# HyTruongSon/GraphFlow

Hardware: AMD Instinct MI355X
Metric: CCN-2D (SMP_omega) molecules/sec fwd+bwd (higher is better)
Workload: dtype f32 (level block products: 2xf16-split operands, 22-bit, fp32 accumulate); 1 GPU; cfg3: SMP_omega 3 levels, C=64, F=5, D=5, cap=29, batch=1024 synthetic QM9-size molecules/GPU, device-resident, fused levels; parallelism=single GPU

## Files before the change

graphflow_amd/csrc/smp_level_c64_split.hip:

```cpp
#include <cstdlib>
#include <type_traits>

#include "gemm_lds.h"
#include "gf_internal.h"
#include "smp_internal.h"

namespace gf {
namespace {

using lds_image::f16v;
using lds_image::f4v;
typedef _Float16 h8 __attribute__((ext_vector_type(8)));
typedef _Float16 h2 __attribute__((ext_vector_type(2)));
typedef float f2v __attribute__((ext_vector_type(2)));

constexpr int kSpThreads = 512;

template <unsigned EMIN = 14u>
__device__ __forceinline__ void pow2_scale(unsigned maxbits, float *s, float *inv) {
    unsigned e = maxbits >> 23;
    e = e < EMIN ? EMIN : e;
    *s = __uint_as_float((267u - e) << 23);
    *inv = __uint_as_float((e - 13u) << 23);
}
// ... 458 lines not shown
    float *facs = winv + 16;
    const int tid = threadIdx.x, lane = tid & 63, li = lane & 31, lh = lane >> 5, wave = tid >> 6;
    for (int t = tid; t < NPOS * E; t += kSmThreads) {
        const int g = (pos0 + t / E) * 512 + t % E;
        imgH[t] = wimg[g];
        imgL[t] = wimg[kSpAll + g];
    }
    if (tid < NPOS) winv[tid] = reinterpret_cast<const float *>(wimg + 2 * kSpAll)[pos0 + tid];
    __syncthreads();
    float *myfac = facs + wave * 32;
    struct Raw {
        f4v a[VPL / 4];
    };
    struct Spl {
        uint4 h[NC], l[NC];
    };
    auto split_blk = [&](const Raw &R, Spl &S, float &inv) {
        unsigned m = 0u;
#pragma unroll
        for (int q = 0; q < VPL / 4; ++q)
#pragma unroll
            for (int j = 0; j < 4; ++j) {
                const unsigned b = __float_as_uint(R.a[q][j]) & 0x7fffffffu;
                m = b > m ? b : m;
            }
        const unsigned mo = (unsigned)__shfl_xor((int)m, 32);
        m = mo > m ? mo : m;
        float sc;
        pow2_scale(m, &sc, &inv);
#pragma unroll
        for (int c = 0; c < NC; ++c) {
            unsigned hw[4], lw[4];
#pragma unroll
            for (int j = 0; j < 4; ++j) {
                h2 h, l;
                const f4v v = R.a[2 * c + (j >> 1)];
                split_pair(v[2 * (j & 1)], v[2 * (j & 1) + 1], sc, &h, &l);
                hw[j] = __builtin_bit_cast(unsigned, h);
                lw[j] = __builtin_bit_cast(unsigned, l);
            }
            S.h[c] = make_uint4(hw[0], hw[1], hw[2], hw[3]);
            S.l[c] = make_uint4(lw[0], lw[1], lw[2], lw[3]);
        }
    };
    auto prod = [&](const Spl &S, float rowfac, int wpos, f16v &acc0, f16v &acc1) {
        __builtin_amdgcn_wave_barrier();
        myfac[li] = rowfac * winv[wpos];
        __builtin_amdgcn_wave_barrier();
        const uint4 *bh = imgH + (size_t)wpos * E + lane, *bl = imgL + (size_t)wpos * E + lane;
#pragma unroll
        for (int nh = 0; nh < NH; ++nh) {
            f16v t;
#pragma unroll
            for (int r = 0; r < 16; ++r) t[r] = 0.f;
#pragma unroll
            for (int c = 0; c < NC; ++c) {
                const h8 bhc = __builtin_bit_cast(h8, bh[(NC * nh + c) * 64]), blc = __builtin_bit_cast(h8, bl[(NC * nh + c) * 64]);
                const h8 ah = __builtin_bit_cast(h8, S.h[c]), al = __builtin_bit_cast(h8, S.l[c]);
                t = __builtin_amdgcn_mfma_f32_32x32x16_f16(al, bhc, t, 0, 0, 0);
                t = __builtin_amdgcn_mfma_f32_32x32x16_f16(ah, blc, t, 0, 0, 0);
            }
#pragma unroll
            for (int r = 0; r < 16; ++r) t[r] *= kLowUnscale;
#pragma unroll
            for (int c = 0; c < NC; ++c) {
                const h8 bhc = __builtin_bit_cast(h8, bh[(NC * nh + c) * 64]);
                const h8 ah = __builtin_bit_cast(h8, S.h[c]);
                t = __builtin_amdgcn_mfma_f32_32x32x16_f16(ah, bhc, t, 0, 0, 0);
            }
            f16v &acc = nh ? acc1 : acc0;
#pragma unroll
            for (int g = 0; g < 4; ++g) {
                const f4v fac = *reinterpret_cast<const f4v *>(myfac + 8 * g + 4 * lh);
#pragma unroll
                for (int j = 0; j < 4; ++j) acc[4 * g + j] += t[4 * g + j] * fac[j];
            }
        }
        __builtin_amdgcn_wave_barrier();
    };
    const int npanels = (rows + 31) / 32;
    for (int p = wg * (kSmThreads / 64) + wave; p < npanels; p += nwg * (kSmThreads / 64)) {
        const int r0 = p * 32;
        const int row = r0 + li < rows ? r0 + li : rows - 1;
        Raw R[NIN];
#pragma unroll
        for (int k = 0; k < NIN; ++k) {
            const float *src = In + (size_t)row * LDA + k * CB + VPL * lh;
#pragma unroll
            for (int q = 0; q < VPL / 4; ++q) R[k].a[q] = *reinterpret_cast<const f4v *>(src + 4 * q);
        }
        (void)NIN;
        auto store_out = [&](int o, const f16v &acc0, const f16v &acc1) {
            float *out = Out + (size_t)(r0 + 4 * lh) * LDOUT + o * CB + li;
#pragma unroll
            for (int r = 0; r < 16; ++r) {
                const int rr = (r & 3) + 8 * (r >> 2);
                if (r0 + 4 * lh + rr < rows && li < CB) {
                    out[(size_t)rr * LDOUT] = acc0[r];
                    if constexpr (NH == 2) out[(size_t)rr * LDOUT + 32] = acc1[r];
                }
            }
        };
        f16v acc0, acc1;
        Spl X;
        float iX;
        if constexpr (PROG == 0) {
#pragma unroll
            for (int r = 0; r < 16; ++r) acc0[r] = acc1[r] = 0.f;
#pragma unroll
            for (int k = 0; k < NPOS; ++k) {
                split_blk(R[k], X, iX);
                prod(X, iX, k, acc0, acc1);
            }
            store_out(0, acc0, acc1);
        } else if constexpr (PROG == 1) {
            split_blk(R[0], X, iX);
#pragma unroll
            for (int k = 0; k < NPOS; ++k) {
#pragma unroll
                for (int r = 0; r < 16; ++r) acc0[r] = acc1[r] = 0.f;
                prod(X, iX, k, acc0, acc1);
                store_out(k, acc0, acc1);
            }
        } else {
#pragma unroll
            for (int k = 0; k < NPOS; ++k) {
                split_blk(R[k], X, iX);
#pragma unroll
                for (int r = 0; r < 16; ++r) acc0[r] = acc1[r] = 0.f;
                prod(X, iX, k, acc0, acc1);
                store_out(k, acc0, acc1);
            }
        }
    }
}

template <int CB>
__global__ __launch_bounds__(kSmThreads, 2) void smp_small_split(SmallJobs jobs, const uint4 *__restrict__ wimg) {
    int j = 0;
    if (jobs.n > 1 && (int)blockIdx.x >= jobs.wg0[1]) j = 1;
    if (jobs.n > 2 && (int)blockIdx.x >= jobs.wg0[2]) j = 2;
    const int wg = (int)blockIdx.x - jobs.wg0[j];
    switch (jobs.prog[j]) {
        case 0: small_split_body<0, CB>(jobs.In[j], jobs.Out[j], jobs.rows[j], wimg, jobs.pos0[j], wg, jobs.nwg[j]); break;
        case 1: small_split_body<1, CB>(jobs.In[j], jobs.Out[j], jobs.rows[j], wimg, jobs.pos0[j], wg, jobs.nwg[j]); break;
        default: small_split_body<2, CB>(jobs.In[j], jobs.Out[j], jobs.rows[j], wimg, jobs.pos0[j], wg, jobs.nwg[j]); break;
    }
}

constexpr int kWsThreads = 512, kWsSlice = 16, kWsRowWords = 12;
constexpr int kWsACols = 256, kWsBCols = 320;
constexpr int kWsStageWords = 2 * (kWsACols + kWsBCols) * kWsRowWords;
constexpr size_t kWsLds = 2 * (size_t)kWsStageWords * 4 + 2 * (kWsACols + kWsBCols) * sizeof(float);
__constant__ int c_ws_ablk[8] = {0, 1, 0, 2, 3, 0, 1, 0};
__constant__ int c_ws_bblk[8] = {1, 1, 2, 0, 0, 3, 3, 4};

__global__ __launch_bounds__(kWsThreads, 1) void smp_wgrad_split(const float *__restrict__ T, const float *__restrict__ dO,
                                                                  const float *__restrict__ rs, int rows, int kchunk,
                                                                  float *__restrict__ part, const int *__restrict__ trow,
                                                                  const unsigned *__restrict__ cmax,
                                                                  const unsigned *__restrict__ chan,
                                                                  float smax, float max_tot, float max_tr,
                                                                  const unsigned *__restrict__ row_max,
                                                                  int packed) {
    extern __shared__ __attribute__((aligned(16))) unsigned ws_smem[];
    const int tid = threadIdx.x, lane = tid & 63, li = lane & 31, lg = lane >> 5;
    const int wave = __builtin_amdgcn_readfirstlane(tid >> 6);
    const int kend = rows;
    auto K = [&](int n) { return (long long)(blockIdx.x + (long long)n * gridDim.x) * kWsSlice; };

    float *sScale = reinterpret_cast<float *>(ws_smem + 2 * kWsStageWords), *sInv = sScale + kWsACols + kWsBCols;
    if (cmax) {
        for (int c = tid; c < kWsACols + kWsBCols; c += kWsThreads) pow2_scale_col(cmax[c], &sScale[c], &sInv[c]);
    } else {
        if (row_max) {
            max_tot = __uint_as_float(row_max[0]);
            max_tr = __uint_as_float(row_max[1]);
        }
        for (int c = tid; c < kWsACols + kWsBCols; c += kWsThreads) {
            const bool isa = c < kWsACols;
            const int blk = (isa ? c : c - kWsACols) >> 6, ch = c & 63;
            const float m = __uint_as_float(chan[(isa ? 0 : 64) + ch]);
            const float fa = blk < 2 ? smax : max_tot;
            const float fb = blk == 0 ? 1.f : blk == 2 ? max_tr : max_tot;
            pow2_scale_col(__float_as_uint(m * (isa ? fa : fb)), &sScale[c], &sInv[c]);
        }
    }
    __syncthreads();

    const int q_lo = lane & 7, pair = lane >> 3;
    struct Task {
        f4v v0, v1;
    };
    constexpr int NB = 2;
    struct Set {
        Task ta, tb[NB];
        float f0[NB], f1[NB];
    };
    const bool has_b1 = wave < 2;
    const int zbit = ((wave >> 1) & 1) == 0 ? 31 : 29;
    const int a_quad = 8 * wave + q_lo;
    auto b_blk = [&](int e) { return (wave + 8 * e) >> 1; };
    auto b_quad = [&](int e) { return 8 * ((wave + 8 * e) & 1) + q_lo; };
    const int rot = (q_lo >> 1) & 3;
    f4v a_scale, b_scale[NB];
#pragma unroll
    for (int i = 0; i < 4; ++i) {
        a_scale[i] = sScale[4 * a_quad + ((i + rot) & 3)];
#pragma unroll
        for (int e = 0; e < NB; ++e) {
            const int blk = b_blk(e) < 5 ? b_blk(e) : 0;
            b_scale[e][i] = sScale[kWsACols + 64 * blk + 4 * b_quad(e) + ((i + rot) & 3)];
        }
    }
    int ia0 = 0, ia1 = 0, ib0 = 0, ib1 = 0;
    auto fetch_trow = [&](int m, int &t0, int &t1) {
        const long long k = K(m) + 2 * pair, last = kend - 1;
        t0 = trow[k < last ? k : last];
        t1 = trow[k + 1 < last ? k + 1 : last];
    };
    auto load_slice = [&](Set &S, int m) {
        const int g0 = packed ? (ia0 & 0x1fffffff) : ia0, g1 = packed ? (ia1 & 0x1fffffff) : ia1;
        const bool z0 = packed && !((ia0 >> zbit) & 1), z1 = packed && !((ia1 >> zbit) & 1);
        const bool zg0 = packed && ia0 >= 0, zg1 = packed && ia1 >= 0;
        ia0 = ib0, ia1 = ib1;
        fetch_trow(m + 2, ib0, ib1);
        const long long last = kend - 1, kk = K(m) + 2 * pair;
        const int c0 = (int)(kk < last ? kk : last), c1 = (int)(kk + 1 < last ? kk + 1 : last);
        const float *t0 = T + (size_t)c0 * 256 + 4 * a_quad, *t1 = T + (size_t)c1 * 256 + 4 * a_quad;
        S.ta.v0 = gf_ld_s<4>(reinterpret_cast<const f4v *>(z0 ? sp_zero_page + 4 * q_lo : t0));
        S.ta.v1 = gf_ld_s<4>(reinterpret_cast<const f4v *>(z1 ? sp_zero_page + 4 * q_lo : t1));
#pragma unroll
        for (int e = 0; e < NB; ++e) {
            const int blk = b_blk(e);
            S.f0[e] = rs[(size_t)c0 * 2 + (blk == 2)];
            S.f1[e] = rs[(size_t)c1 * 2 + (blk == 2)];
            const bool gathered = blk == 4;
            const float *src = blk < 5 ? dO + (blk >= 3 ? 64 : 0) + 4 * b_quad(e) : T + 4 * a_quad;
            const int ld = blk < 5 ? 128 : 256;
            const float *s0 = src + (size_t)(gathered ? g0 : c0) * ld, *s1 = src + (size_t)(gathered ? g1 : c1) * ld;
            S.tb[e].v0 = gf_ld_s<256>(reinterpret_cast<const f4v *>((gathered && zg0) ? sp_zero_page + 4 * q_lo : s0));
            S.tb[e].v1 = gf_ld_s<256>(reinterpret_cast<const f4v *>((gathered && zg1) ? sp_zero_page + 4 * q_lo : s1));
        }
    };
    auto rotate = [&](f4v v) {
        if (rot & 1) v = f4v{v[1], v[2], v[3], v[0]};
        if (rot & 2) v = f4v{v[2], v[3], v[0], v[1]};
        return v;
    };
    auto store_task = [&](const f4v &v0, const f4v &v1, unsigned *H, unsigned *L, int col0, const f4v &sc, float f0, float f1) {
        const f4v r0 = rotate(v0), r1 = rotate(v1);
#pragma unroll
        for (int i = 0; i < 4; ++i) {
            h2 h, l;
            split_plain2(r0[i], r1[i], sc[i] * f0, sc[i] * f1, &h, &l);
            const int w = (col0 + ((i + rot) & 3)) * kWsRowWords + pair;
            H[w] = __builtin_bit_cast(unsigned, h);
            L[w] = __builtin_bit_cast(unsigned, l);
        }
    };
    auto store_slice = [&](const Set &S, long long k0, unsigned *stage) {
        unsigned *Ah = stage, *Al = Ah + kWsACols * kWsRowWords, *Bh = Al + kWsACols * kWsRowWords, *Bl = Bh + kWsBCols * kWsRowWords;
        const long long k = k0 + 2 * pair;
        const float ok0 = k < kend ? 1.f : 0.f, ok1 = k + 1 < kend ? 1.f : 0.f;
        store_task(S.ta.v0, S.ta.v1, Ah, Al, 4 * a_quad, a_scale, ok0, ok1);
#pragma unroll
        for (int e = 0; e < NB; ++e) {
            if (e == 1 && !has_b1) break;
            const int blk = b_blk(e);
            const bool scaled = blk == 1 || blk == 2;
            const float m0 = scaled ? S.f0[e] : 1.f, m1 = scaled ? S.f1[e] : 1.f;
            store_task(S.tb[e].v0, S.tb[e].v1, Bh, Bl, 64 * blk + 4 * b_quad(e), b_scale[e], ok0 * m0, ok1 * m1);
        }
    };

    f16v acc[2][2];
#pragma unroll
    for (int r = 0; r < 16; ++r) acc[0][0][r] = acc[0][1][r] = acc[1][0][r] = acc[1][1][r] = 0.f;
    const int ablk = c_ws_ablk[wave], bblk = c_ws_bblk[wave];
    auto products = [&](const unsigned *stage) {
        const unsigned *Ah = stage, *Al = Ah + kWsACols * kWsRowWords, *Bh = Al + kWsACols * kWsRowWords, *Bl = Bh + kWsBCols * kWsRowWords;
        const int ao = (ablk * 64 + li) * kWsRowWords + 4 * lg, bo = (bblk * 64 + li) * kWsRowWords + 4 * lg;
        h8 ah[2], al[2], bh[2], bl[2];
#pragma unroll
        for (int t = 0; t < 2; ++t) {
            ah[t] = __builtin_bit_cast(h8, *reinterpret_cast<const uint4 *>(Ah + ao + t * 32 * kWsRowWords));
            al[t] = __builtin_bit_cast(h8, *reinterpret_cast<const uint4 *>(Al + ao + t * 32 * kWsRowWords));
            bh[t] = __builtin_bit_cast(h8, *reinterpret_cast<const uint4 *>(Bh + bo + t * 32 * kWsRowWords));
            bl[t] = __builtin_bit_cast(h8, *reinterpret_cast<const uint4 *>(Bl + bo + t * 32 * kWsRowWords));
        }
#pragma unroll
        for (int mt = 0; mt < 2; ++mt)
#pragma unroll
            for (int nt = 0; nt < 2; ++nt) {
                acc[mt][nt] = __builtin_amdgcn_mfma_f32_32x32x16_f16(al[mt], bh[nt], acc[mt][nt], 0, 0, 0);
                acc[mt][nt] = __builtin_amdgcn_mfma_f32_32x32x16_f16(ah[mt], bl[nt], acc[mt][nt], 0, 0, 0);
                acc[mt][nt] = __builtin_amdgcn_mfma_f32_32x32x16_f16(ah[mt], bh[nt], acc[mt][nt], 0, 0, 0);
            }
    };
    auto interval = [&](Set &Ra, int n) {
        store_slice(Ra, K(n + 1), ws_smem + ((n + 1) & 1) * kWsStageWords);
        load_slice(Ra, n + 4);
        products(ws_smem + (n & 1) * kWsStageWords);
        __syncthreads();
    };
    if (K(0) < kend) {
        Set S0, S1, S2;
        fetch_trow(0, ia0, ia1);
        fetch_trow(1, ib0, ib1);
        load_slice(S0, 0);
        load_slice(S1, 1);
        load_slice(S2, 2);
        store_slice(S0, K(0), ws_smem);
        load_slice(S0, 3);
        __syncthreads();
        int left = (int)((kend - K(0) + (long long)gridDim.x * kWsSlice - 1) / ((long long)gridDim.x * kWsSlice));
        int n = 0;
        for (; left >= 3; n += 3, left -= 3) {
            interval(S1, n);
            interval(S2, n + 1);
            interval(S0, n + 2);
        }
        if (left >= 1) interval(S1, n);
        if (left >= 2) interval(S2, n + 1);
    }
    float *out = part + ((size_t)blockIdx.x * 8 + wave) * 4096 + li;
    const float *ia = sInv + ablk * 64, *ib = sInv + kWsACols + bblk * 64;
#pragma unroll
    for (int mt = 0; mt < 2; ++mt)
#pragma unroll
        for (int nt = 0; nt < 2; ++nt) {
            const float ub = ib[32 * nt + li];
#pragma unroll
            for (int r = 0; r < 16; ++r) {
                const int row = 32 * mt + (r & 3) + 8 * (r >> 2) + 4 * lg;
                out[row * 64 + 32 * nt] = acc[mt][nt][r] * (ia[row] * ub);
            }
        }
}


constexpr long long kTrowWindow = (long long)kFusedMaxField * kFusedMaxField;
constexpr int kW8Threads = 256;
template <int CB, int NF, int NX = 0>
__global__ __launch_bounds__(kW8Threads, 1) void smp_wgrad_all(const float *__restrict__ T, const float *__restrict__ dO,
                                                                const float *__restrict__ rs, int rows, float *__restrict__ part,
                                                                const int *__restrict__ trow, const unsigned *__restrict__ cmax,
                                                                const unsigned *__restrict__ chan, float smax,
                                                                const unsigned *__restrict__ row_max, int packed, float *__restrict__ xpart = nullptr) {
    static_assert(CB == 32 || CB == 16, "one 32 x 32 tile per product");
    static_assert(NX == 0 || (NX == 3 && NF == 2), "the extra products take the plain (tot, tr) row factors");
    constexpr int NP = 8 + NX;
    constexpr int ACOLS = 4 * CB, BCOLS = 5 * CB;
    constexpr int SL = CB == 16 ? 2 * kWsSlice : kWsSlice;
    constexpr int TROW = 16 * CB, DROW = 8 * CB;
    constexpr int NBF = NF == 8 ? 8 : 5;
    __shared__ float sScale[ACOLS + BCOLS], sInv[ACOLS + BCOLS];
    __shared__ float sImg[NP * CB * CB];
    const int tid = threadIdx.x, lane = tid & 63, li = lane & 31, lg = lane >> 5;
    const int wave = __builtin_amdgcn_readfirstlane(tid >> 6);
    const int hi = (CB == 16 && li >= 16) ? 1 : 0;
    const int lc = CB == 16 ? (li & 15) : li;
    const int rb = 8 * lg + 16 * hi;
    if (cmax) {
        for (int c = tid; c < ACOLS + BCOLS; c += kW8Threads) pow2_scale_col(cmax[c], &sScale[c], &sInv[c]);
    } else {
        const float max_tot = __uint_as_float(row_max[0]), max_tr = __uint_as_float(row_max[1]);
        for (int c = tid; c < ACOLS + BCOLS; c += kW8Threads) {
            const bool isa = c < ACOLS;
            const int blk = (isa ? c : c - ACOLS) / CB, ch = c % CB;
            const float m = __uint_as_float(chan[(isa ? 0 : CB) + ch]);
            const float fa = blk < 2 ? smax : max_tot;
            const float fb = blk == 0 ? 1.f : blk == 2 ? max_tr : max_tot;
            pow2_scale_col(__float_as_uint(m * (isa ? fa : fb)), &sScale[c], &sInv[c]);
        }
    }
    __syncthreads();
    float sa[4], sb[5];
#pragma unroll
    for (int k = 0; k < 4; ++k) sa[k] = sScale[CB * k + lc];
#pragma unroll
    for (int k = 0; k < 5; ++k) sb[k] = sScale[ACOLS + CB * k + lc];

    constexpr int kOut = 0x40000000;
    const long long nsl = ((long long)rows + SL - 1) / SL;
    auto slice_of = [&](int m) { return (long long)blockIdx.x + ((long long)wave + 4ll * m) * gridDim.x; };
    struct Idx {
        int t[8];
    };
    struct Fac {
        float f[8][NF == 8 ? 8 : 2];
    };
    struct Raw {
        float a[4][8], l[8], u[8], g[8];
    };
    const __amdgpu_buffer_rsrc_t rTr = __builtin_amdgcn_make_buffer_rsrc(const_cast<int *>(trow), 0, (unsigned)rows * 4u, 0x00020000);
    constexpr int rsb = 4 * NF;
    const __amdgpu_buffer_rsrc_t rRs = __builtin_amdgcn_make_buffer_rsrc(const_cast<float *>(rs), 0, (unsigned)rows * (unsigned)rsb, 0x00020000);
    auto ld1 = [](__amdgpu_buffer_rsrc_t r, int voff, int soff) {
        return __builtin_bit_cast(float, __builtin_amdgcn_raw_buffer_load_b32(r, voff, soff, 0));
    };
    typedef int i4v __attribute__((ext_vector_type(4)));
    auto first_row = [&](int m) {
        const long long k0 = slice_of(m) * SL;
        return k0 < rows ? (int)k0 : rows;
    };
    auto load_idx = [&](Idx &I, int m) {
        const int ks = first_row(m);
        const i4v t0 = __builtin_bit_cast(i4v, __builtin_amdgcn_raw_buffer_load_b128(rTr, 4 * rb, ks * 4, 0));
        const i4v t1 = __builtin_bit_cast(i4v, __builtin_amdgcn_raw_buffer_load_b128(rTr, 4 * rb + 16, ks * 4, 0));
        I.t[0] = t0[0], I.t[1] = t0[1], I.t[2] = t0[2], I.t[3] = t0[3], I.t[4] = t1[0], I.t[5] = t1[1], I.t[6] = t1[2], I.t[7] = t1[3];
    };
    auto load_fac = [&](Fac &F, int m) {
        const int ks = first_row(m);
#pragma unroll
        for (int q = 0; q < 8 * NF / 4; ++q) {
            const f4v v = __builtin_bit_cast(f4v, __builtin_amdgcn_raw_buffer_load_b128(rRs, rsb * rb + 16 * q, ks * rsb, 0));
#pragma unroll
            for (int e = 0; e < 4; ++e) F.f[(4 * q + e) / NF][(4 * q + e) % NF] = v[e];
        }
    };
    auto load_raw = [&](Raw &R, const Idx &I, int m) {
        const long long k0 = slice_of(m) * SL;
        const bool live = k0 < rows;
        long long left = (long long)rows - k0;
        left = left < 0 ? 0 : left > SL ? SL : left;
        const long long k0c = live ? k0 : 0;
        const __amdgpu_buffer_rsrc_t rT = __builtin_amdgcn_make_buffer_rsrc(const_cast<float *>(T + (size_t)k0c * ACOLS), 0, (unsigned)(left * TROW), 0x00020000);
        const long long g0 = k0c > kTrowWindow ? k0c - kTrowWindow : 0;
        long long g1 = k0c + SL + kTrowWindow;
        g1 = g1 > rows ? rows : g1;
        const __amdgpu_buffer_rsrc_t rD = __builtin_amdgcn_make_buffer_rsrc(const_cast<float *>(dO + (size_t)g0 * 2 * CB), 0, live ? (unsigned)((g1 - g0) * DROW) : 0u, 0x00020000);
        const int own = (int)(k0c - g0) * DROW;
        const int ig0 = (int)g0;
        const int offA = rb * TROW + lc * 4, offL = rb * DROW + lc * 4, offU = offL + CB * 4;
#pragma unroll
        for (int j = 0; j < 8; ++j) {
            const int t = I.t[j];
            const bool p31 = !packed || ((t >> 31) & 1), p29 = !packed || ((t >> 29) & 1);
            const int v31 = p31 ? offA : kOut, v29 = p29 ? offA : kOut;
            const int tr = packed ? (t & 0x1fffffff) : t;
            const int vg = p31 ? (tr - ig0) * DROW + (CB + lc) * 4 : kOut;
            R.a[0][j] = ld1(rT, v31, j * TROW);
            R.a[1][j] = ld1(rT, v29 + CB * 4, j * TROW);
            R.a[2][j] = ld1(rT, v31 + 2 * CB * 4, j * TROW);
            R.a[3][j] = ld1(rT, v29 + 3 * CB * 4, j * TROW);
            R.l[j] = ld1(rD, offL, own + j * DROW);
            R.u[j] = ld1(rD, offU, own + j * DROW);
            R.g[j] = ld1(rD, vg, 0);
        }
    };
    f16v acc[NP];
#pragma unroll
    for (int p = 0; p < NP; ++p)
#pragma unroll
        for (int r = 0; r < 16; ++r) acc[p][r] = 0.f;
    auto frag = [&](const float (&v)[8], float sc, const Fac *F, int col, h8 *H, h8 *L) {
        unsigned hw[4], lw[4];
#pragma unroll
        for (int i = 0; i < 4; ++i) {
            h2 h, l;
            split_plain2(v[2 * i], v[2 * i + 1], F ? sc * F->f[2 * i][col] : sc, F ? sc * F->f[2 * i + 1][col] : sc, &h, &l);
            hw[i] = __builtin_bit_cast(unsigned, h);
            lw[i] = __builtin_bit_cast(unsigned, l);
        }
        *H = __builtin_bit_cast(h8, make_uint4(hw[0], hw[1], hw[2], hw[3]));
        *L = __builtin_bit_cast(h8, make_uint4(lw[0], lw[1], lw[2], lw[3]));
    };
    constexpr int kA[11] = {0, 1, 0, 2, 3, 0, 1, 0, 0, 1, 1}, kB[11] = {1, 1, 2, 0, 0, 3, 3, 4, 0, 0, 2};
    const long long first = (long long)blockIdx.x + (long long)wave * gridDim.x;
    if (first < nsl) {
        const int mine = (int)((nsl - first + 4ll * gridDim.x - 1) / (4ll * gridDim.x));
        Idx I0, I1;
        Fac F0, F1;
        Raw R0, R1;
        load_idx(I0, 0);
        load_idx(I1, 1);
// ... 162 lines not shown
                                                               long long rows1, int ld1, int C, unsigned *__restrict__ out) {
    __shared__ unsigned red[64];
    const float *X = blockIdx.y ? X1 : X0;
    const long long rows = blockIdx.y ? rows1 : rows0;
    const int ld = blockIdx.y ? ld1 : ld0, nq = C / 4, rpb = 256 / nq;
    if (threadIdx.x < 64) red[threadIdx.x] = 0u;
    __syncthreads();
    const int q = threadIdx.x % nq, rr = threadIdx.x / nq;
    f4v m = {0.f, 0.f, 0.f, 0.f};
    if (rr < rpb)
        for (long long r = (long long)blockIdx.x * rpb + rr; r < rows; r += (long long)gridDim.x * rpb) {
            const f4v v = *reinterpret_cast<const f4v *>(X + (size_t)r * ld + 4 * q);
#pragma unroll
            for (int j = 0; j < 4; ++j) m[j] = fmaxf(m[j], fabsf(v[j]));
        }
#pragma unroll
    for (int j = 0; j < 4; ++j) atomicMax(&red[4 * q + j], __float_as_uint(m[j]));
    __syncthreads();
    if ((int)threadIdx.x < C && red[threadIdx.x]) atomicMax(&out[C * blockIdx.y + threadIdx.x], red[threadIdx.x]);
}
__global__ void rowscale_absmax(const float *__restrict__ rs, int rows, unsigned *__restrict__ out) {
    float a = 0.f, b = 0.f;
    for (int r = blockIdx.x * blockDim.x + threadIdx.x; r < rows; r += gridDim.x * blockDim.x) {
        a = fmaxf(a, fabsf(rs[2 * (size_t)r]));
        b = fmaxf(b, fabsf(rs[2 * (size_t)r + 1]));
    }
    atomicMax(&out[0], __float_as_uint(a));
    atomicMax(&out[1], __float_as_uint(b));
}
__global__ void wgrad_bounds_exact(const unsigned *__restrict__ mt, const unsigned *__restrict__ mo, const unsigned *__restrict__ mx,
                                   unsigned *__restrict__ cmax) {
    const int c = threadIdx.x;
    const float tot = __uint_as_float(mx[0]), tr = __uint_as_float(mx[1]);
#pragma unroll
    for (int k = 0; k < 4; ++k) cmax[64 * k + c] = mt[64 * k + c];
    const float l = __uint_as_float(mo[c]), u = __uint_as_float(mo[64 + c]);
    cmax[kWsACols + c] = __float_as_uint(l);
    cmax[kWsACols + 64 + c] = __float_as_uint(tot * l);
    cmax[kWsACols + 128 + c] = __float_as_uint(tr * l);
    cmax[kWsACols + 192 + c] = cmax[kWsACols + 256 + c] = __float_as_uint(u);
}

}

bool smp_split_products(const gf_ctx *ctx) {
    if (ctx && ctx->fp32_products) return false;
    return !env_is("GF_SMP_SPLIT", '0');
}

static bool packed_rows(const int *trowf, int rows, int row_limit) {
    return trowf && rows < row_limit && !env_is("GF_SMP_MASK_ZEROS", '0');
}

size_t smp_split_image_bytes() { return 2 * (size_t)kSpImgStride * sizeof(uint4); }
template <int C>
static gf_status launch_small_split(gf_ctx *ctx, const char *name, int total, size_t lds, const SmallJobs &jb, const uint4 *img) {
    gf_status st = opt_in_lds(ctx, smp_small_split<C>, lds);
    if (st != GF_OK) return st;
    GF_LAUNCH(ctx, name, smp_small_split<C>, dim3((unsigned)total), dim3(kSmThreads), lds, jb, img);
    return GF_OK;
}
gf_status smp_small_split_c64(gf_ctx *ctx, bool transposed, int n, const int *prog, const float *const *In, float *const *Out, const int *rows,
                              const int *pos0, const void *wimg, const char *name, int C) {
    const uint4 *img = static_cast<const uint4 *>(wimg) + (transposed ? kSpImgStride : 0);
    SmallJobs jb;
    jb.n = 0;
    int total = 0;
    for (int j = 0; j < n && jb.n < 3; ++j) {
        if (rows[j] < 1) continue;
        const int npanels = (rows[j] + 31) / 32, per = kSmThreads / 64, want = (npanels + per - 1) / per;
        const int k = jb.n++;
        jb.In[k] = In[j], jb.Out[k] = Out[j], jb.rows[k] = rows[j], jb.pos0[k] = pos0[j], jb.prog[k] = prog[j];
        jb.wg0[k] = total;
        jb.nwg[k] = want < 512 ? want : 512;
        total += jb.nwg[k];
    }
    if (total == 0) return GF_OK;
    const size_t lds = 2 * (size_t)4 * (C >= 32 ? C / 32 : 1) * (C / 16) * 64 * 16 + 16 * sizeof(float) + (kSmThreads / 64) * 32 * sizeof(float);
    switch (C) {
    case 16: return launch_small_split<16>(ctx, name, total, lds, jb, img);
    case 32: return launch_small_split<32>(ctx, name, total, lds, jb, img);
    case 64: return launch_small_split<64>(ctx, name, total, lds, jb, img);
    }
    return fail(ctx, GF_ERR_UNSUPPORTED, "smp_small_split: %d channels", C);
}

gf_status smp_split_build_images(gf_ctx *ctx, const float *const *Wst, void *const *img, int n, int C, const float *const *X) {
    for (int i0 = 0; i0 < n; i0 += kSpImgLevels) {
        SplitImages a;
        const int m = n - i0 < kSpImgLevels ? n - i0 : kSpImgLevels;
        for (int i = 0; i < m; ++i) {
            a.Wst[i] = Wst[i0 + i];
            a.X[i] = X ? X[i0 + i] : nullptr;
            a.img[i] = static_cast<uint4 *>(img[i0 + i]);
        }
        GF_LAUNCH(ctx, "smpf_stack_w", smp_split_weight_images, dim3(2, m, kSpPos), dim3(kSpThreads), 0, a, C);
    }
    return GF_OK;
}

struct RowpanelArgs {
    int grid;
    const float *A, *rowscale, *Wst;
    float *Out;
    int rows;
    const int *trow;
    int store_mask;
    const uint4 *img;
};
template <bool F, bool M, int CB, int NF, int NX>
static gf_status launch_rowpanel_split(gf_ctx *ctx, const RowpanelArgs &a) {
    const size_t lds = 2 * (size_t)(8 + NX) * (CB >= 32 ? CB / 32 : 1) * (CB / 16) * 64 * 16 + 32 * sizeof(float) + (kSpThreads / 64) * 32 * sizeof(float);
    gf_status st = opt_in_lds(ctx, smp_rowpanel_split<F, M, CB, NF, NX>, lds);
    if (st != GF_OK) return st;
    GF_LAUNCH(ctx, F ? "smpf_products_fwd" : "smpf_products_bwd", (smp_rowpanel_split<F, M, CB, NF, NX>), dim3((unsigned)a.grid), dim3(kSpThreads),
              lds, a.A, a.rowscale, a.Wst, a.Out, a.rows, a.trow, a.store_mask, a.img);
    return GF_OK;
}
template <int CB, int NF, int NX = 0>
static gf_status launch_rowpanel_split(gf_ctx *ctx, bool forward, bool mask, const RowpanelArgs &a) {
    if (forward) return mask ? launch_rowpanel_split<true, true, CB, NF, NX>(ctx, a) : launch_rowpanel_split<true, false, CB, NF, NX>(ctx, a);
    return mask ? launch_rowpanel_split<false, true, CB, NF, NX>(ctx, a) : launch_rowpanel_split<false, false, CB, NF, NX>(ctx, a);
}

gf_status smp_rowpanel_split_c64(gf_ctx *ctx, bool forward, const float *A, const float *rowscale, const float *Wst, float *Out,
                                 int rows, const int *trow, int cus, const int *trowf, bool skip_zero_grads, const void *wimg, int C, int nf, int nx) {
    const int per = kSpThreads / 64;
    const int npanels = (rows + 31) / 32;
    const int want = (npanels + per - 1) / per;
    const int slots = C == 64 ? cus : 2 * cus;
    const int grid = want < slots ? want : slots;
    if (C != 64 && !wimg) return fail(ctx, GF_ERR_UNSUPPORTED, "smp_rowpanel_split: %d channels need the level's prebuilt weight images", C);
    const bool mask = packed_rows(trowf, rows, 1 << 29);
    const RowpanelArgs a = {grid, A, rowscale, Wst, Out, rows, mask ? trowf : trow, skip_zero_grads ? 1 : 0,
                            wimg ? static_cast<const uint4 *>(wimg) + (forward ? 0 : kSpImgStride) : nullptr};
    if (nx != 0) {
        if (nx != 3 || nf != 2 || !(C == 32 || C == 16) || !wimg)
            return fail(ctx, GF_ERR_UNSUPPORTED, "smp_rowpanel_split: %d extra products at %d channels / %d row factors", nx, C, nf);
        return C == 32 ? launch_rowpanel_split<32, 2, 3>(ctx, forward, mask, a) : launch_rowpanel_split<16, 2, 3>(ctx, forward, mask, a);
    }
    if (nf != 2 && !(nf == 8 && (C == 32 || C == 16))) return fail(ctx, GF_ERR_UNSUPPORTED, "smp_rowpanel_split: %d row factors at %d channels", nf, C);
    if (nf == 8)
        return C == 32 ? launch_rowpanel_split<32, 8>(ctx, forward, mask, a) : launch_rowpanel_split<16, 8>(ctx, forward, mask, a);
    switch (C) {
    case 64: return launch_rowpanel_split<64, 2>(ctx, forward, mask, a);
    case 32: return launch_rowpanel_split<32, 2>(ctx, forward, mask, a);
    case 16: return launch_rowpanel_split<16, 2>(ctx, forward, mask, a);
    }
    return fail(ctx, GF_ERR_UNSUPPORTED, "smp_rowpanel_split: %d channels", C);
}

gf_status smp_wgrad_partials_split_c64(gf_ctx *ctx, const float *T, const float *dO, const float *rowscale, int rows, int kchunk,
                                       int splits, float *part, const int *trow, const WgradScales &ws, const int *trowf) {
    gf_status st = opt_in_lds(ctx, smp_wgrad_split, kWsLds);
    if (st != GF_OK) return st;
    const bool mask = packed_rows(trowf, rows, 1 << 29);
    GF_LAUNCH(ctx, "smpf_wgrad", smp_wgrad_split, dim3((unsigned)splits), dim3(kWsThreads), kWsLds, T, dO, rowscale, rows, kchunk, part,
              mask ? trowf : trow, ws.cmax, ws.chan, ws.smax, ws.max_tot, ws.max_tr, ws.row_max, mask ? 1 : 0);
    return GF_OK;
}


template <int CB>
static gf_status launch_wgrad_all(gf_ctx *ctx, const float *T, const float *dO, const float *rowscale, int rows, int splits, float *part,
                                  const int *tr, const unsigned *cmax, const unsigned *chan, float smax, const unsigned *row_max, int packed, int nf,
                                  float *xpart = nullptr) {
    if (xpart) {
        if (nf != 2) return fail(ctx, GF_ERR_UNSUPPORTED, "smp_wgrad_all: extra products with %d row factors", nf);
        GF_LAUNCH(ctx, "smpf_wgrad", (smp_wgrad_all<CB, 2, 3>), dim3((unsigned)splits), dim3(kW8Threads), 0, T, dO, rowscale, rows, part, tr, cmax, chan, smax,
                  row_max, packed, xpart);
    } else if (nf == 8) {
        GF_LAUNCH(ctx, "smpf_wgrad", (smp_wgrad_all<CB, 8>), dim3((unsigned)splits), dim3(kW8Threads), 0, T, dO, rowscale, rows, part, tr, cmax, chan, smax,
                  row_max, packed);
    } else {
        GF_LAUNCH(ctx, "smpf_wgrad", (smp_wgrad_all<CB, 2>), dim3((unsigned)splits), dim3(kW8Threads), 0, T, dO, rowscale, rows, part, tr, cmax, chan, smax,
                  row_max, packed);
    }
    return GF_OK;
}
gf_status smp_wgrad_partials_all(gf_ctx *ctx, const float *T, const float *dO, const float *rowscale, int rows, int splits, float *part,
                                  const int *trow, const int *trowf, unsigned *words, const unsigned *chan, float smax,
                                  const unsigned *row_max, int nf, int C, float *xpart) {
    const bool mask = packed_rows(trowf, rows, 1 << 28);
    const int *tr = mask ? trowf : trow;
    if (C == 16) {
        if (chan && row_max)
            return launch_wgrad_all<16>(ctx, T, dO, rowscale, rows, splits, part, tr, (const unsigned *)nullptr, chan, smax, row_max, mask ? 1 : 0, nf, xpart);
        if (nf != 2) return fail(ctx, GF_ERR_UNSUPPORTED, "smp_wgrad_all: exact column bounds with per-product row factors");
        GF_HIP_TRY(ctx, hipMemsetAsync(words, 0, sizeof(unsigned) * 512, ctx->stream));
        const long long g0 = ((long long)rows + 63) / 64;
        const unsigned g = (unsigned)(g0 < 1 ? 1 : g0 > 256 ? 256 : g0);
        GF_LAUNCH(ctx, "smpf_colmax", level_channel_maxima_ld, dim3(g, 1), dim3(256), 0, T, (long long)rows, 64, (const float *)nullptr, 0ll, 0, 64, words);
        GF_LAUNCH(ctx, "smpf_colmax", level_channel_maxima_ld, dim3(g, 1), dim3(256), 0, dO, (long long)rows, 32, (const float *)nullptr, 0ll, 0, 32, words + 256);
        GF_LAUNCH(ctx, "smpf_colmax", rowscale_absmax, dim3(64), dim3(256), 0, rowscale, rows, words + 384);
        GF_LAUNCH(ctx, "smpf_colmax", wgrad_bounds_exact_cb, dim3(1), dim3(64), 0, words, words + 256, words + 384, words + 512, 16);
        return launch_wgrad_all<16>(ctx, T, dO, rowscale, rows, splits, part, tr, words + 512, (const unsigned *)nullptr, 0.f, (const unsigned *)nullptr, mask ? 1 : 0, nf, xpart);
    }
    if (C != 32) return fail(ctx, GF_ERR_UNSUPPORTED, "smp_wgrad_all: %d channels", C);
    constexpr int CB = 32;
    if (chan && row_max)
        return launch_wgrad_all<CB>(ctx, T, dO, rowscale, rows, splits, part, tr, (const unsigned *)nullptr, chan, smax, row_max, mask ? 1 : 0, nf, xpart);
    GF_HIP_TRY(ctx, hipMemsetAsync(words, 0, sizeof(unsigned) * 512, ctx->stream));
    const long long g0 = ((long long)rows + 15) / 16;
    const unsigned g = (unsigned)(g0 < 1 ? 1 : g0 > 1024 ? 1024 : g0);
    for (int k = 0; k < 4 * CB / 64; ++k) GF_LAUNCH(ctx, "smpf_colmax", col_absmax64, dim3(g), dim3(256), 0, T + 64 * k, (long long)rows, 4 * CB, words + 64 * k);
    for (int k = 0; k < 2 * CB / 64; ++k) GF_LAUNCH(ctx, "smpf_colmax", col_absmax64, dim3(g), dim3(256), 0, dO + 64 * k, (long long)rows, 2 * CB, words + 256 + 64 * k);
    if (nf != 2) return fail(ctx, GF_ERR_UNSUPPORTED, "smp_wgrad_all: exact column bounds with per-product row factors");
    GF_LAUNCH(ctx, "smpf_colmax", rowscale_absmax, dim3(64), dim3(256), 0, rowscale, rows, words + 384);
    GF_LAUNCH(ctx, "smpf_colmax", wgrad_bounds_exact_cb, dim3(1), dim3(64), 0, words, words + 256, words + 384, words + 512, CB);
    return launch_wgrad_all<CB>(ctx, T, dO, rowscale, rows, splits, part, tr, words + 512, (const unsigned *)nullptr, 0.f, (const unsigned *)nullptr, mask ? 1 : 0, nf, xpart);
}
size_t smp_wgrad_all_words() { return 512 + 9 * 32; }
int smp_wgrad_all_splits(gf_ctx *ctx, long long rows) {
    static int cu_count[64] = {};
    const int di = ctx->device & 63;
    if (!cu_count[di]) {
        if (hipDeviceGetAttribute(&cu_count[di], hipDeviceAttributeMultiprocessorCount, ctx->device) != hipSuccess || cu_count[di] < 1) cu_count[di] = 256;
    }
    const long long cap = cu_count[di];
    const long long slices = (rows + 15) / 16, want = slices / 8;
    return (int)(want < 1 ? 1 : want > cap ? cap : want);
}

size_t smp_wgrad_bound_words() { return 128; }
gf_status smp_wgrad_channel_maxima(gf_ctx *ctx, const float *fprev, long long prev_rows, const float *dsrc, long long drows, unsigned *words) {
    const long long big = prev_rows > drows ? prev_rows : drows, g0 = (big + 63) / 64;
    const unsigned g = (unsigned)(g0 < 1 ? 1 : g0 > 256 ? 256 : g0);
    GF_LAUNCH(ctx, "smpf_colmax", level_channel_maxima, dim3(g, 2), dim3(256), 0, fprev, prev_rows, dsrc, drows, words);
    return GF_OK;
}
gf_status smp_wgrad_channel_maxima_ld(gf_ctx *ctx, const float *fprev, long long prev_rows, int ld0, const float *dsrc, long long drows, int ld1, int C,
                                      unsigned *words) {
    const long long big = prev_rows > drows ? prev_rows : drows, g0 = (big + 63) / 64;
    const unsigned g = (unsigned)(g0 < 1 ? 1 : g0 > 256 ? 256 : g0);
    GF_LAUNCH(ctx, "smpf_colmax", level_channel_maxima_ld, dim3(g, 2), dim3(256), 0, fprev, prev_rows, ld0, dsrc, drows, ld1, C, words);
    return GF_OK;
}
size_t smp_wgrad_bound_words_exact() { return 512 + kWsACols + kWsBCols; }
gf_status smp_wgrad_column_bounds_exact(gf_ctx *ctx, const float *T, const float *dO, const float *rowscale, int rows, unsigned *words) {
    GF_HIP_TRY(ctx, hipMemsetAsync(words, 0, sizeof(unsigned) * 512, ctx->stream));
    const long long g0 = ((long long)rows + 15) / 16;
    const unsigned g = (unsigned)(g0 < 1 ? 1 : g0 > 1024 ? 1024 : g0);
    for (int k = 0; k < 4; ++k) GF_LAUNCH(ctx, "smpf_colmax", col_absmax64, dim3(g), dim3(256), 0, T + 64 * k, (long long)rows, 256, words + 64 * k);
    for (int k = 0; k < 2; ++k) GF_LAUNCH(ctx, "smpf_colmax", col_absmax64, dim3(g), dim3(256), 0, dO + 64 * k, (long long)rows, 128, words + 256 + 64 * k);
    GF_LAUNCH(ctx, "smpf_colmax", rowscale_absmax, dim3(64), dim3(256), 0, rowscale, rows, words + 384);
    GF_LAUNCH(ctx, "smpf_colmax", wgrad_bounds_exact, dim3(1), dim3(64), 0, words, words + 256, words + 384, words + 512);
    return GF_OK;
}

}
```

Measured before the change: 159,200 molecules/s.

## Restructure wgrad split loader around buffer loads with per-lane row fragments

Rewrites the staging loader of the split-precision weight-gradient kernel. Each lane now owns one column and eight consecutive rows. Loads go through buffer resources whose out-of-range offsets return zero, replacing the zero-page pointer redirection and the clamped indices. Row-scale factors are broadcast across lanes with DPP, and the split halves are written to LDS as 128-bit stores instead of scattered 32-bit stores. The loop tail is replaced by an unconditional loop that relies on bounds-checked zeros for dead slices. This adds a 2 GiB limit on dO and depends on the out-of-range offset encoding.

```diff
diff --git a/graphflow_amd/csrc/smp_level_c64_split.hip b/graphflow_amd/csrc/smp_level_c64_split.hip
--- a/graphflow_amd/csrc/smp_level_c64_split.hip
+++ b/graphflow_amd/csrc/smp_level_c64_split.hip
@@ -634,6 +634,15 @@
 constexpr int kWsACols = 256, kWsBCols = 320;
 constexpr int kWsStageWords = 2 * (kWsACols + kWsBCols) * kWsRowWords;
 constexpr size_t kWsLds = 2 * (size_t)kWsStageWords * 4 + 2 * (kWsACols + kWsBCols) * sizeof(float);
+template <int N>
+__device__ __forceinline__ float row_bcast(float v) {
+    return __builtin_bit_cast(float, __builtin_amdgcn_update_dpp(0, __builtin_bit_cast(int, v), 0x150 + N, 0xf, 0xf, false));
+}
+template <int COL>
+__device__ __forceinline__ void row_factors(float f, float sc, float (&out)[8]) {
+    out[0] = sc * row_bcast<COL>(f), out[1] = sc * row_bcast<2 + COL>(f), out[2] = sc * row_bcast<4 + COL>(f), out[3] = sc * row_bcast<6 + COL>(f);
+    out[4] = sc * row_bcast<8 + COL>(f), out[5] = sc * row_bcast<10 + COL>(f), out[6] = sc * row_bcast<12 + COL>(f), out[7] = sc * row_bcast<14 + COL>(f);
+}
 __constant__ int c_ws_ablk[8] = {0, 1, 0, 2, 3, 0, 1, 0};
 __constant__ int c_ws_bblk[8] = {1, 1, 2, 0, 0, 3, 3, 4};
 
@@ -670,89 +679,108 @@
     }
     __syncthreads();
 
-    const int q_lo = lane & 7, pair = lane >> 3;
-    struct Task {
-        f4v v0, v1;
-    };
-    constexpr int NB = 2;
+    constexpr int kOut = (int)0xC0000000u;
+    constexpr int TROW = 1024, DROW = 512;
+    constexpr int kAuxT = (GF_NT_SITES & 4) != 0 ? 2 : 0;
+    typedef int i4v __attribute__((ext_vector_type(4)));
+    const int rb = 8 * lg;
+    const int zmask = ((wave >> 1) & 1) == 0 ? (int)0x80000000u : 0x20000000;
+    const int unpacked = packed ? 0 : -1, trmask = packed ? 0x1fffffff : -1;
+    enum { kBL = 0, kBdU = 1, kBGather = 2, kBNone = 3 };
+    const int b_kind = wave < 2 ? kBL : wave < 4 ? kBdU : wave < 6 ? kBNone : kBGather;
+    const int b_blk = b_kind == kBL ? 0 : b_kind == kBdU ? 3 : 4;
+    const int b_col = (b_kind == kBL ? 0 : 64) + 32 * (wave & 1) + li;
+    const int a_word = (32 * wave + li) * kWsRowWords + 4 * lg;
+    const int b_word = (64 * b_blk + 32 * (wave & 1) + li) * kWsRowWords + 4 * lg;
+    const float a_scale = sScale[32 * wave + li];
+    float b_scale[3];
+#pragma unroll
+    for (int e = 0; e < 3; ++e) b_scale[e] = sScale[kWsACols + 64 * (b_kind == kBL ? e : b_blk) + 32 * (wave & 1) + li];
     struct Set {
-        Task ta, tb[NB];
-        float f0[NB], f1[NB];
-    };
-    const bool has_b1 = wave < 2;
-    const int zbit = ((wave >> 1) & 1) == 0 ? 31 : 29;
-    const int a_quad = 8 * wave + q_lo;
-    auto b_blk = [&](int e) { return (wave + 8 * e) >> 1; };
-    auto b_quad = [&](int e) { return 8 * ((wave + 8 * e) & 1) + q_lo; };
-    const int rot = (q_lo >> 1) & 3;
-    f4v a_scale, b_scale[NB];
-#pragma unroll
-    for (int i = 0; i < 4; ++i) {
-        a_scale[i] = sScale[4 * a_quad + ((i + rot) & 3)];
-#pragma unroll
-        for (int e = 0; e < NB; ++e) {
-            const int blk = b_blk(e) < 5 ? b_blk(e) : 0;
-            b_scale[e][i] = sScale[kWsACols + 64 * blk + 4 * b_quad(e) + ((i + rot) & 3)];
-        }
-    }
-    int ia0 = 0, ia1 = 0, ib0 = 0, ib1 = 0;
-    auto fetch_trow = [&](int m, int &t0, int &t1) {
-        const long long k = K(m) + 2 * pair, last = kend - 1;
-        t0 = trow[k < last ? k : last];
-        t1 = trow[k + 1 < last ? k + 1 : last];
+        float a[8], b[8];
+        float f;
+    };
+    const __amdgpu_buffer_rsrc_t rTr = __builtin_amdgcn_make_buffer_rsrc(const_cast<int *>(trow), 0, (unsigned)rows * 4u, 0x00020000);
+    const __amdgpu_buffer_rsrc_t rRs =
+        __builtin_amdgcn_make_buffer_rsrc(const_cast<float *>(rs), 0, b_kind == kBL ? (unsigned)rows * 8u : 0u, 0x00020000);
+    const __amdgpu_buffer_rsrc_t rD =
+        __builtin_amdgcn_make_buffer_rsrc(const_cast<float *>(dO), 0, b_kind != kBNone ? (unsigned)rows * (unsigned)DROW : 0u, 0x00020000);
+    auto first_row = [&](int m) {
+        const long long k0 = K(m);
+        return k0 < kend ? (int)k0 : kend;
+    };
+    struct Idx {
+        int t[8];
+    };
+    Idx tn, tn2;
+    auto fetch_trow = [&](int m, Idx &I) {
+        const int ks = first_row(m);
+        const i4v t0 = __builtin_bit_cast(i4v, __builtin_amdgcn_raw_buffer_load_b128(rTr, 4 * rb, ks * 4, 0));
+        const i4v t1 = __builtin_bit_cast(i4v, __builtin_amdgcn_raw_buffer_load_b128(rTr, 4 * rb + 16, ks * 4, 0));
+        I.t[0] = t0[0], I.t[1] = t0[1], I.t[2] = t0[2], I.t[3] = t0[3], I.t[4] = t1[0], I.t[5] = t1[1], I.t[6] = t1[2], I.t[7] = t1[3];
     };
     auto load_slice = [&](Set &S, int m) {
-        const int g0 = packed ? (ia0 & 0x1fffffff) : ia0, g1 = packed ? (ia1 & 0x1fffffff) : ia1;
-        const bool z0 = packed && !((ia0 >> zbit) & 1), z1 = packed && !((ia1 >> zbit) & 1);
-        const bool zg0 = packed && ia0 >= 0, zg1 = packed && ia1 >= 0;
-        ia0 = ib0, ia1 = ib1;
-        fetch_trow(m + 2, ib0, ib1);
-        const long long last = kend - 1, kk = K(m) + 2 * pair;
-        const int c0 = (int)(kk < last ? kk : last), c1 = (int)(kk + 1 < last ? kk + 1 : last);
-        const float *t0 = T + (size_t)c0 * 256 + 4 * a_quad, *t1 = T + (size_t)c1 * 256 + 4 * a_quad;
-        S.ta.v0 = gf_ld_s<4>(reinterpret_cast<const f4v *>(z0 ? sp_zero_page + 4 * q_lo : t0));
-        S.ta.v1 = gf_ld_s<4>(reinterpret_cast<const f4v *>(z1 ? sp_zero_page + 4 * q_lo : t1));
-#pragma unroll
-        for (int e = 0; e < NB; ++e) {
-            const int blk = b_blk(e);
-            S.f0[e] = rs[(size_t)c0 * 2 + (blk == 2)];
-            S.f1[e] = rs[(size_t)c1 * 2 + (blk == 2)];
-            const bool gathered = blk == 4;
-            const float *src = blk < 5 ? dO + (blk >= 3 ? 64 : 0) + 4 * b_quad(e) : T + 4 * a_quad;
-            const int ld = blk < 5 ? 128 : 256;
-            const float *s0 = src + (size_t)(gathered ? g0 : c0) * ld, *s1 = src + (size_t)(gathered ? g1 : c1) * ld;
-            S.tb[e].v0 = gf_ld_s<256>(reinterpret_cast<const f4v *>((gathered && zg0) ? sp_zero_page + 4 * q_lo : s0));
-            S.tb[e].v1 = gf_ld_s<256>(reinterpret_cast<const f4v *>((gathered && zg1) ? sp_zero_page + 4 * q_lo : s1));
-        }
-    };
-    auto rotate = [&](f4v v) {
-        if (rot & 1) v = f4v{v[1], v[2], v[3], v[0]};
-        if (rot & 2) v = f4v{v[2], v[3], v[0], v[1]};
-        return v;
-    };
-    auto store_task = [&](const f4v &v0, const f4v &v1, unsigned *H, unsigned *L, int col0, const f4v &sc, float f0, float f1) {
-        const f4v r0 = rotate(v0), r1 = rotate(v1);
+        const long long k0 = K(m);
+        const bool live = k0 < kend;
+        long long left = (long long)kend - k0;
+        left = left < 0 ? 0 : left > kWsSlice ? kWsSlice : left;
+        const long long k0c = live ? k0 : 0;
+        const __amdgpu_buffer_rsrc_t rT =
+            __builtin_amdgcn_make_buffer_rsrc(const_cast<float *>(T + (size_t)k0c * kWsACols), 0, (unsigned)(left * TROW), 0x00020000);
+        const unsigned own = (unsigned)(live ? k0 : kend) * DROW;
+        const int offA = rb * TROW + (32 * wave + li) * 4, offB = rb * DROW + b_col * 4;
+        int va[8], vb[8];
+#pragma unroll
+        for (int j = 0; j < 8; ++j) {
+            va[j] = ((tn.t[j] & zmask) | unpacked) != 0 ? offA : kOut;
+            vb[j] = offB;
+        }
+        if (b_kind == kBGather) {
+#pragma unroll
+            for (int j = 0; j < 8; ++j) {
+                const int t = tn.t[j];
+                vb[j] = (t | unpacked) < 0 ? (t & trmask) * DROW + b_col * 4 : kOut;
+            }
+        }
+        const unsigned sb0 = b_kind == kBGather ? 0u : own, sbj = b_kind == kBGather ? 0u : (unsigned)DROW;
+        tn = tn2;
+        fetch_trow(m + 2, tn2);
+        const int ks = first_row(m);
+        S.f = __builtin_bit_cast(float, __builtin_amdgcn_raw_buffer_load_b32(rRs, rb * 8 + (lane & 15) * 4, ks * 8, 0));
+#pragma unroll
+        for (int j = 0; j < 8; ++j) {
+            S.a[j] = __builtin_bit_cast(float, __builtin_amdgcn_raw_buffer_load_b32(rT, va[j], j * TROW, kAuxT));
+            S.b[j] = __builtin_bit_cast(float, __builtin_amdgcn_raw_buffer_load_b32(rD, vb[j], sb0 + j * sbj, 0));
+        }
+    };
+    auto store_frag = [&](const float (&v)[8], float sc, float f, auto col, unsigned *H, unsigned *L) {
+        constexpr int COL = decltype(col)::value;
+        float s8[8];
+        if constexpr (COL < 0) {
+#pragma unroll
+            for (int j = 0; j < 8; ++j) s8[j] = sc;
+        } else {
+            row_factors<COL>(f, sc, s8);
+        }
+        unsigned hw[4], lw[4];
 #pragma unroll
         for (int i = 0; i < 4; ++i) {
             h2 h, l;
-            split_plain2(r0[i], r1[i], sc[i] * f0, sc[i] * f1, &h, &l);
-            const int w = (col0 + ((i + rot) & 3)) * kWsRowWords + pair;
-            H[w] = __builtin_bit_cast(unsigned, h);
-            L[w] = __builtin_bit_cast(unsigned, l);
-        }
-    };
-    auto store_slice = [&](const Set &S, long long k0, unsigned *stage) {
+            split_plain2(v[2 * i], v[2 * i + 1], s8[2 * i], s8[2 * i + 1], &h, &l);
+            hw[i] = __builtin_bit_cast(unsigned, h);
+            lw[i] = __builtin_bit_cast(unsigned, l);
+        }
+        *reinterpret_cast<uint4 *>(H) = make_uint4(hw[0], hw[1], hw[2], hw[3]);
+        *reinterpret_cast<uint4 *>(L) = make_uint4(lw[0], lw[1], lw[2], lw[3]);
+    };
+    auto store_slice = [&](const Set &S, unsigned *stage) {
         unsigned *Ah = stage, *Al = Ah + kWsACols * kWsRowWords, *Bh = Al + kWsACols * kWsRowWords, *Bl = Bh + kWsBCols * kWsRowWords;
-        const long long k = k0 + 2 * pair;
-        const float ok0 = k < kend ? 1.f : 0.f, ok1 = k + 1 < kend ? 1.f : 0.f;
-        store_task(S.ta.v0, S.ta.v1, Ah, Al, 4 * a_quad, a_scale, ok0, ok1);
-#pragma unroll
-        for (int e = 0; e < NB; ++e) {
-            if (e == 1 && !has_b1) break;
-            const int blk = b_blk(e);
-            const bool scaled = blk == 1 || blk == 2;
-            const float m0 = scaled ? S.f0[e] : 1.f, m1 = scaled ? S.f1[e] : 1.f;
-            store_task(S.tb[e].v0, S.tb[e].v1, Bh, Bl, 64 * blk + 4 * b_quad(e), b_scale[e], ok0 * m0, ok1 * m1);
+        using std::integral_constant;
+        store_frag(S.a, a_scale, 0.f, integral_constant<int, -1>{}, Ah + a_word, Al + a_word);
+        if (b_kind != kBNone) store_frag(S.b, b_scale[0], 0.f, integral_constant<int, -1>{}, Bh + b_word, Bl + b_word);
+        if (b_kind == kBL) {
+            store_frag(S.b, b_scale[1], S.f, integral_constant<int, 0>{}, Bh + b_word + 64 * kWsRowWords, Bl + b_word + 64 * kWsRowWords);
+            store_frag(S.b, b_scale[2], S.f, integral_constant<int, 1>{}, Bh + b_word + 128 * kWsRowWords, Bl + b_word + 128 * kWsRowWords);
         }
     };
 
@@ -781,30 +809,27 @@
             }
     };
     auto interval = [&](Set &Ra, int n) {
-        store_slice(Ra, K(n + 1), ws_smem + ((n + 1) & 1) * kWsStageWords);
+        store_slice(Ra, ws_smem + ((n + 1) & 1) * kWsStageWords);
         load_slice(Ra, n + 4);
         products(ws_smem + (n & 1) * kWsStageWords);
         __syncthreads();
     };
     if (K(0) < kend) {
         Set S0, S1, S2;
-        fetch_trow(0, ia0, ia1);
-        fetch_trow(1, ib0, ib1);
+        fetch_trow(0, tn);
+        fetch_trow(1, tn2);
         load_slice(S0, 0);
         load_slice(S1, 1);
         load_slice(S2, 2);
-        store_slice(S0, K(0), ws_smem);
+        store_slice(S0, ws_smem);
         load_slice(S0, 3);
         __syncthreads();
         int left = (int)((kend - K(0) + (long long)gridDim.x * kWsSlice - 1) / ((long long)gridDim.x * kWsSlice));
-        int n = 0;
-        for (; left >= 3; n += 3, left -= 3) {
+        for (int n = 0; n < left; n += 3) {
             interval(S1, n);
             interval(S2, n + 1);
             interval(S0, n + 2);
         }
-        if (left >= 1) interval(S1, n);
-        if (left >= 2) interval(S2, n + 1);
     }
     float *out = part + ((size_t)blockIdx.x * 8 + wave) * 4096 + li;
     const float *ia = sInv + ablk * 64, *ib = sInv + kWsACols + bblk * 64;
@@ -1273,6 +1298,7 @@
 
 gf_status smp_wgrad_partials_split_c64(gf_ctx *ctx, const float *T, const float *dO, const float *rowscale, int rows, int kchunk,
                                        int splits, float *part, const int *trow, const WgradScales &ws, const int *trowf) {
+    if ((long long)rows * 512 > 0x7fffffffll) return fail(ctx, GF_ERR_UNSUPPORTED, "smp_wgrad_split: %d rows (dO above 2 GiB)", rows);
     gf_status st = opt_in_lds(ctx, smp_wgrad_split, kWsLds);
     if (st != GF_OK) return st;
     const bool mask = packed_rows(trowf, rows, 1 << 29);
```

Result: no change. 160,800 molecules/s (median of 6 runs) (+1.0%).
